# Xharlie/BtcDet

Hardware: AMD Instinct MI355X
Metric: scenes/s fwd+bwd KITTI-Car bs=2/GPU (BtcDet hot path) (higher is better)
Workload: dtype f32

## Files before the change

btcdet_amd/_lib.py:

```python
import ctypes
import os

import numpy as np
import torch

_HERE = os.path.dirname(os.path.abspath(__file__))
LIB_PATH = os.path.join(_HERE, "libbtcdet_hip.so")
_lib = None

c_i32p = ctypes.POINTER(ctypes.c_int32)
c_f32p = ctypes.POINTER(ctypes.c_float)
vp = ctypes.c_void_p
ci = ctypes.c_int
sz = ctypes.c_size_t

MODE_SUBM, MODE_CONV, MODE_TRANSPOSE = 0, 1, 2


class BtcHipError(RuntimeError):
    pass


class BtcOccConfig(ctypes.Structure):
    _fields_ = [("batch", ctypes.c_int32), ("grid", ctypes.c_int32 * 3), ("sphere_grid", ctypes.c_int32 * 3),
# ... 74 lines not shown
    "btc_conv_bf16w_supported": (ci, [ci, ci, ci]),
    "btc_weights_to_bf16": (ci, [vp, ci, ci, ci, vp, vp, vp]),
    "btc_conv_split_supported": (ci, [ci, ci, ci]),
    "btc_set_scratch": (ci, [vp, vp, sz]),
    "btc_conv_split_wanted": (ci, [ci, ci, ci, ci]),
    "btc_weights_split3": (ci, [vp, ci, ci, ci, vp, vp, vp]),
    "btc_weights_split3_multi": (ci, [vp, vp, vp, c_i32p, c_i32p, c_i32p, ci, vp]),
    "btc_weights_to_bf16_multi": (ci, [vp, vp, vp, c_i32p, c_i32p, c_i32p, ci, vp]),
    "btc_conv_fwd_bf16w": (ci, [vp, vp, vp, vp, ci, ci, ci, ci, vp, vp]),
    "btc_conv_dgrad_bf16w": (ci, [vp, vp, vp, ci, ci, ci, ci, vp, vp]),
    "btc_row_orders": (ci, [vp, c_i32p, c_i32p, ci, vp, vp]),
    "btc_row_orders_keyed": (ci, [vp, vp, c_i32p, c_i32p, ci, vp, vp]),
    "btc_conv_apply_ordered": (ci, [ci, ci, vp, vp, vp, vp, vp, ci, ci, ci, ci, vp, vp]),
    "btc_conv_apply_src": (ci, [ci, ci, vp, ctypes.c_longlong, vp, vp, vp, vp, ci, ci, ci, ci, vp, vp]),
    "btc_conv_wgrad_ordered": (ci, [ci, vp, vp, vp, ci, vp, ci, vp, vp, ci, ci, ci, vp, vp, sz, vp]),
    "btc_conv_wgrad_slabs": (ci, [ci, vp, vp, vp, ci, vp, ci, vp, vp, ci, ci, ci, vp, vp, sz, vp, vp]),
    "btc_wgrad_reduce_multi": (ci, [vp, vp, vp, vp, ci, vp]),
    "btc_adam_group_ws_bytes": (sz, [ci]),
    "btc_adam_max_segments": (ci, []),
    "btc_grads_pack": (ci, [vp, ci, vp, vp, vp, vp, c_i32p, vp, vp]),
    "btc_adam_group_step": (ci, [vp, ci, vp, vp, vp, vp, c_i32p, ci, vp, vp, vp, ctypes.c_longlong, ctypes.c_float, ctypes.c_float, ctypes.c_float,
                                 ctypes.c_float, ctypes.c_float, ctypes.c_float, vp, sz, vp]),
    "btc_maxpool_fwd": (ci, [vp, vp, ci, ci, ci, vp, vp]),
    "btc_maxpool_bwd": (ci, [vp, vp, vp, vp, ci, ci, ci, vp, vp]),
    "btc_dense_fwd": (ci, [vp, vp, ci, ci, c_i32p, vp, vp]),
    "btc_dense_bwd": (ci, [vp, vp, ci, ci, c_i32p, vp, vp]),
    "btc_revoxelize_ws_bytes": (sz, [ci, ci, c_i32p]),
    "btc_revoxelize_count": (ci, [vp, ci, ci, c_i32p, vp, vp, vp, sz, vp]),
    "btc_revoxelize_fill": (ci, [vp, vp, ci, ci, ci, c_i32p, ci, ci, vp, vp, vp, vp, sz, vp]),
    "btc_pass_occ_vox_ws_bytes": (sz, [ctypes.POINTER(BtcPovConfig), ci, ci]),
    "btc_pass_occ_vox_count": (ci, [ctypes.POINTER(BtcPovConfig), vp, vp, vp, vp, vp, vp, ci, ci, ci, vp, vp, sz, vp]),
    "btc_pass_occ_vox_fill": (ci, [ctypes.POINTER(BtcPovConfig), vp, ci, ci, ci, ci, ci, ci, vp, vp, vp, vp, vp, vp, sz, vp]),
    "btc_pass_occ_vox_fill_i32": (ci, [ctypes.POINTER(BtcPovConfig), vp, ci, ci, ci, ci, ci, ci, vp, vp, vp, vp, vp, vp, vp, vp, sz, vp]),
    "btc_occ_loss_ws_bytes": (sz, []),
    "btc_occ_loss_fwd": (ci, [vp, vp, vp, vp, vp, vp, vp, vp, ci, ctypes.c_longlong, ctypes.c_float, ctypes.c_float, ctypes.c_float, vp, vp, vp,
                              sz, vp]),
    "btc_occ_loss_bwd": (ci, [vp, vp, vp, vp, vp, vp, vp, vp, ci, ctypes.c_longlong, ctypes.c_float, vp, vp, vp, vp, vp]),
    "btc_occ_loss_fwd_total": (ci, [vp, vp, vp, vp, vp, vp, vp, vp, ci, ctypes.c_longlong, ctypes.c_float, ctypes.c_float, ctypes.c_float, vp, vp,
                                    vp, sz, vp]),
    "btc_occ_loss_bwd_total": (ci, [vp, vp, vp, vp, vp, vp, vp, vp, ci, ctypes.c_longlong, ctypes.c_float, vp, vp, vp, vp, vp]),
    "btc_dense_split_fwd": (ci, [vp, vp, ci, ci, ci, vp, vp, vp, vp]),
    "btc_occ_prob": (ci, [vp, vp, ci, ctypes.c_longlong, vp, vp]),
    "btc_dense_split_bwd": (ci, [vp, vp, vp, ci, ci, ci, vp, vp, vp]),
    "btc_cat_pad_fwd": (ci, [vp, ci, vp, ci, ctypes.c_longlong, ci, ci, vp, vp]),
    "btc_cat_pad_bwd": (ci, [vp, ci, ctypes.c_longlong, ci, vp, ci, vp, ci, vp]),
    "btc_sumsq2_ws_bytes": (sz, []),
    "btc_sumsq2_fwd": (ci, [vp, ctypes.c_longlong, ci, ctypes.c_double, vp, ctypes.c_longlong, ci, ctypes.c_double, vp, vp, sz, vp]),
    "btc_sumsq2_bwd": (ci, [vp, ctypes.c_longlong, ci, ctypes.c_float, vp, vp, ctypes.c_longlong, ci, ctypes.c_float, vp, vp, vp]),
    "btc_bn_ws_bytes": (sz, [ci]),
    "btc_bn_relu_fwd": (ci, [vp, ci, ci, vp, vp, vp, vp, vp, ctypes.c_float, ctypes.c_float, ci, ci, vp, vp, vp, vp, sz, vp]),
    "btc_spin": (ci, [ci, vp]),
    "btc_bn_relu_bwd": (ci, [vp, vp, vp, ci, ci, vp, vp, vp, ci, ci, vp, vp, vp, vp, sz, vp]),
    "btc_bn_relu_fwd_bf16": (ci, [vp, ci, ci, vp, vp, vp, vp, vp, ctypes.c_float, ctypes.c_float, ci, ci, vp, vp, vp, vp, sz, vp]),
    "btc_bn_relu_bwd_bf16": (ci, [vp, vp, vp, ci, ci, vp, vp, vp, ci, ci, vp, vp, vp, vp, sz, vp]),
    "btc_ball_query": (ci, [vp, vp, vp, vp, ci, ci, ctypes.c_float, ctypes.c_float, ci, vp, vp]),
    "btc_group_points": (ci, [vp, vp, vp, vp, ci, ci, ci, ci, vp, vp]),
    "btc_group_points_grad": (ci, [vp, vp, vp, vp, ci, ci, ci, ci, ci, vp, vp]),
    "btc_furthest_point_sampling": (ci, [vp, ci, ci, ci, vp, vp, vp]),
    "btc_three_nn": (ci, [vp, vp, vp, vp, ci, ci, vp, vp, vp]),
    "btc_three_interpolate": (ci, [vp, vp, vp, ci, ci, vp, vp]),
    "btc_three_interpolate_grad": (ci, [vp, vp, vp, ci, ci, ci, vp, vp]),
    "btc_bn_fuse_ws_bytes": (sz, []),
    "btc_conv_bn_relu_fwd": (ci, [ci, vp, vp, vp, vp, vp, ci, ci, ci, ci, vp, vp, vp, vp, vp, vp, ctypes.c_float, ctypes.c_float, ci, vp, vp, vp, vp, sz, vp, vp]),
    "btc_conv_bn_relu_fwd_src": (ci, [ci, vp, ctypes.c_longlong, vp, vp, vp, vp, ci, ci, ci, ci, vp, vp, vp, vp, vp, vp, ctypes.c_float, ctypes.c_float, ci, vp, vp, vp, vp, sz, vp, vp]),
    "btc_col_sum": (ci, [vp, ci, ci, vp, vp, sz, vp]),
    "btc_col_sum_bf16": (ci, [vp, ci, ci, vp, vp, sz, vp]),
    "btc_occ_targets_ws_bytes": (sz, [ctypes.POINTER(BtcOccConfig)]),
    "btc_occ_backproject_lut": (ci, [ctypes.POINTER(BtcOccConfig), vp, vp]),
    "btc_occ_targets": (ci, [ctypes.POINTER(BtcOccConfig), vp, vp, vp, ci, ci, ci, vp, vp, vp, vp, ci, vp, vp,
                             ctypes.POINTER(BtcOccBuffers), vp, sz, vp]),
}

EXPORTED_SYMBOLS = tuple(_SIGS.keys())

_INFER_SIGS = {
    "btc_conv_bn_eval_fwd": (ci, [ci, vp, ctypes.c_longlong, vp, vp, vp, vp, ci, ci, ci, ci, vp, vp, vp, vp, ctypes.c_float, ci, vp, vp]),
    "btc_det_select_nms_ws_bytes": (sz, [ci, ci]),
    "btc_det_select_nms": (ci, [vp, vp, ci, ci, ci, ci, ci, ctypes.c_float, ctypes.c_float, ci, ci, ci, vp, vp, vp, vp, sz, vp]),
    "btc_det_finish": (ci, [vp, vp, ci, ci, ci, ci, ci, ci, vp, vp, vp, vp, ci, vp, ci, ci, vp, ci, ci, c_f32p, ci, vp, vp, vp, vp, vp, vp]),
    "btc_kitti_overlaps": (ci, [vp, vp, vp, vp, vp, c_i32p, ci, vp, vp, vp]),
    "btc_kitti_match_tp": (ci, [vp, vp, vp, vp, vp, vp, vp, c_i32p, ci, ci, ci, ci, ci, ci, vp, vp, vp]),
    "btc_kitti_match_stats_ws_bytes": (sz, [ci, ci, ci, ci, ci]),
    "btc_kitti_match_stats": (ci, [vp, vp, vp, vp, vp, vp, vp, vp, vp, vp, vp, c_i32p, ci, ci, ci, ci, ci, ci, ci, vp, vp, vp, sz, vp]),
}

INFER_EXPORTED_SYMBOLS = tuple(_INFER_SIGS.keys())


def lib():
    global _lib
    if _lib is None:
        if not os.path.exists(LIB_PATH):
            raise BtcHipError(
                f"{LIB_PATH} not found: build it with `python -c 'import __graft_entry__ as g; g.build()'` "
                f"or `make -C btcdet_amd/csrc` (there is no CPU fallback for the hot path)")
        L = ctypes.CDLL(LIB_PATH)
        for name, (res, args) in list(_SIGS.items()) + list(_INFER_SIGS.items()):
            fn = getattr(L, name)
            fn.restype = res
            fn.argtypes = args
        for kv in filter(None, os.environ.get("BTC_TUNE", "").split(",")):
            k, v = kv.split("=")
            if L.btc_tune_set(int(k), int(v)) != 0:
                raise BtcHipError("BTC_TUNE: bad entry %r" % kv)
        _lib = L
    return _lib


_fast = False


def fast():
    global _fast
    if _fast is False:
        _fast = None
        if os.environ.get("BTC_FASTPATH", "1") != "0":
            try:
                lib()
                from . import _btcfast
                if _btcfast.abi_version() == lib().btc_version():
                    _fast = _btcfast
            except ImportError:
                _fast = None
    return _fast


def check(rc, what):
    if rc != 0:
        msg = lib().btc_last_error().decode("utf-8", "replace")
        raise BtcHipError(f"{what} failed (code {rc}): {msg}")


_raw_stream = torch._C._cuda_getCurrentRawStream
_cur_device = torch._C._cuda_getDevice


def stream_ptr():
    return _raw_stream(_cur_device())


def ptr(t):
    if t is None:
        return None
    if not (t.is_cuda and t.is_contiguous()):
        raise BtcHipError("expected a contiguous tensor on the GPU (HIP) device")
    return t.data_ptr()


_I3_CACHE = {}


def i3(v):
    if isinstance(v, (int, np.integer)):
        key = (int(v),) * 3
    else:
        key = tuple(int(x) for x in np.asarray(v).reshape(-1))
        if len(key) != 3:
            raise BtcHipError(f"expected 3 values, got {v!r}")
    a = _I3_CACHE.get(key)
    if a is None:
        a = np.ascontiguousarray(np.array(key, dtype=np.int32))
        a.setflags(write=False)
        a_ptr = a.ctypes.data_as(c_i32p)
        _I3_CACHE[key] = a
        _I3P_CACHE[id(a)] = (a, a_ptr)
    return a
# ... 19 lines not shown
```

btcdet_amd/csrc/btc_common.h:

```cpp
#pragma once
#include <hip/hip_runtime.h>
#include <stdint.h>
#include <stdio.h>

#include "../../include/btcdet_hip.h"

#define BTC_EMPTY_KEY (-1)
#define BTC_EMPTY_IDX 0x7F7F7F7F

void btc_set_error(const char* fmt, ...);

#define BTC_CHECK_ARG(cond, ...)            \
  do {                                      \
    if (!(cond)) {                          \
      btc_set_error(__VA_ARGS__);           \
      return BTC_EINVAL;                    \
    }                                       \
  } while (0)

#define BTC_HIP(call)                                                             \
  do {                                                                            \
    hipError_t e_ = (call);                                                       \
    if (e_ != hipSuccess) {                                                       \
      btc_set_error("%s failed: %s (%s:%d)", #call, hipGetErrorString(e_), __FILE__, __LINE__); \
      return BTC_ELAUNCH;                                                         \
    }                                                                             \
  } while (0)

#define BTC_LAUNCH_CHECK()                                                        \
  do {                                                                            \
    hipError_t e_ = hipGetLastError();                                            \
    if (e_ != hipSuccess) {                                                       \
      btc_set_error("kernel launch failed: %s (%s:%d)", hipGetErrorString(e_), __FILE__, __LINE__); \
      return BTC_ELAUNCH;                                                         \
    }                                                                             \
  } while (0)

#if defined(__HIP_DEVICE_COMPILE__) && !defined(__gfx950__)
#error "the fence-free last-arriver protocol (btc_ticket_take) is derived for gfx950's sc1 write-through stores only"
#endif
#if defined(__HIPCC__)
template <class T>
__device__ __forceinline__ void btc_st_agent(T* p, T v) { __hip_atomic_store(p, v, __ATOMIC_RELAXED, __HIP_MEMORY_SCOPE_AGENT); }
template <class T>
__device__ __forceinline__ T btc_ld_agent(const T* p) { return __hip_atomic_load(p, __ATOMIC_RELAXED, __HIP_MEMORY_SCOPE_AGENT); }
__device__ __forceinline__ int btc_ticket_take(int32_t* counter) {
  asm volatile("s_waitcnt vmcnt(0)" ::: "memory");
  return __hip_atomic_fetch_add(counter, 1, __ATOMIC_RELAXED, __HIP_MEMORY_SCOPE_AGENT);
}
__device__ __forceinline__ void btc_ticket_acquire() { __builtin_amdgcn_fence(__ATOMIC_ACQUIRE, "agent"); }
#endif

#define BTC_TUNE_KEYS 24
int btc_tune_get(int key);

bool btc_apply_glds_supported(int K, int Cred, int Cres);
bool btc_apply_glds_has_shape(int shape, bool bf = false);
size_t btc_apply_glds_lds_bytes(int shape, int kc, int K, bool bf, int stages = 3);
int btc_apply_glds_stages(int shape, int kc, int K, bool bf, int asked);
int btc_launch_apply_glds(bool trans_w, int shape, int kc, int xcd, bool bf, const void* feat, const float* W, const float* bias,
                          const int32_t* nbr, const int32_t* order , int n_rows, int K, int Cred, int Cres, void* out,
                          hipStream_t stream, const struct BnFuse* bn = nullptr );

int btc_apply(const char* who, int pass, int operands, const void* src, long long src_rows, const void* W, const float* bias, const int32_t* nbr,
              const int32_t* order, int n_rows, int K, int Cin, int Cout, void* dst, hipStream_t stream, const struct BnFuse* bn);

int btc_apply_bf16w(const void* src, const void* Wq, const float* bias, const int32_t* nbr, const int32_t* order, int n_rows, int K, int Cred,
                    int Cres, void* dst, hipStream_t stream, int mirror = 0, const struct BnFuse* bn = nullptr);
bool btc_wgrad_x_supported(int mode, int K, int cg, int cc);
int btc_wgrad_x_plan(int mode, int rows, int K, int cg, int cc, int* S, int* ph, int* z = nullptr);
int btc_launch_wgrad_x(int mode, const void* g, const void* c, const int32_t* map, const int32_t* ord, int rows, int K, int cg, int cc, float* part,
                       int swap, hipStream_t stream);
int btc_wgrad_n_kind(int K, int Cin, int Cout);
int btc_wgrad_n_plan(int rows);
int btc_launch_wgrad_n(bool bf, const void* walked, const void* gathered, const int32_t* map, int rows, int K, int Cw, int Cn, float* part,
                       int flags , hipStream_t stream);
constexpr size_t BTC_SCRATCH_HEAD = 64 * 1024;
constexpr long long BTC_SCRATCH_TICKETS = BTC_SCRATCH_HEAD / 4;
void* btc_scratch(hipStream_t stream, size_t* bytes);
struct BnFuse;
int btc_apply_split(const float* src, const void* Ws, const float* bias, const int32_t* nbr, const int32_t* order, int n_rows, int K, int Cred,
                    int Cres, float* dst, hipStream_t stream, int mirror, const BnFuse* bn);

__host__ __device__ __forceinline__ unsigned short btc_f32_to_bf16(float f) {
  union { float f; unsigned u; } c;
  c.f = f;
  unsigned u = c.u;
  if ((u & 0x7fffffffu) > 0x7f800000u) return (unsigned short)((u >> 16) | 0x40);
  u += 0x7fffu + ((u >> 16) & 1u);
  return (unsigned short)(u >> 16);
}
__host__ __device__ __forceinline__ float btc_bf16_to_f32(unsigned short h) {
  union { float f; unsigned u; } c;
  c.u = (unsigned)h << 16;
  return c.f;
}

template <bool BF>
__device__ __forceinline__ float4 btc_ld4(const float* base, size_t i) {
  if (!BF) return *reinterpret_cast<const float4*>(base + i);
  const uint2 v = *reinterpret_cast<const uint2*>(reinterpret_cast<const unsigned short*>(base) + i);
  return make_float4(__uint_as_float(v.x << 16), __uint_as_float(v.x & 0xffff0000u), __uint_as_float(v.y << 16),
                     __uint_as_float(v.y & 0xffff0000u));
}
template <bool BF>
__device__ __forceinline__ float btc_ld1(const float* base, size_t i) {
  if (!BF) return base[i];
  return __uint_as_float((unsigned)reinterpret_cast<const unsigned short*>(base)[i] << 16);
}
template <bool BF>
__device__ __forceinline__ void btc_st4(float* base, size_t i, float a, float b, float c, float d) {
  if (!BF) {
    *reinterpret_cast<float4*>(base + i) = make_float4(a, b, c, d);
  } else {
    uint2 v;
    v.x = (unsigned)btc_f32_to_bf16(a) | ((unsigned)btc_f32_to_bf16(b) << 16);
    v.y = (unsigned)btc_f32_to_bf16(c) | ((unsigned)btc_f32_to_bf16(d) << 16);
    *reinterpret_cast<uint2*>(reinterpret_cast<unsigned short*>(base) + i) = v;
  }
}
template <bool BF>
__device__ __forceinline__ void btc_st1(float* base, size_t i, float a) {
  if (!BF) base[i] = a;
  else reinterpret_cast<unsigned short*>(base)[i] = btc_f32_to_bf16(a);
}

#ifdef __cplusplus
#include <mutex>
constexpr int BTC_MAX_DEVICES = 16;
struct BtcPerDeviceOnce {
  std::once_flag flag[BTC_MAX_DEVICES];
};
template <class F>
static inline void btc_once_per_device(BtcPerDeviceOnce& o, F&& fn) {
  int dev = 0;
  (void)hipGetDevice(&dev);
  std::call_once(o.flag[dev >= 0 && dev < BTC_MAX_DEVICES ? dev : 0], fn);
}
#endif

typedef float f32x4 __attribute__((ext_vector_type(4)));
constexpr int TM = 64;
__host__ __device__ constexpr int ldb_of(int nt) { return nt * 16 + (((nt * 16) % 32 == 0) ? 16 : 0); }

static inline int btc_cdiv(long long a, long long b) { return (int)((a + b - 1) / b); }
static inline size_t btc_align(size_t x, size_t a = 256) { return (x + a - 1) / a * a; }
static inline unsigned btc_pow2_ge(unsigned long long v) {
  unsigned long long p = 1;
// ... 40 lines not shown
```

btcdet_amd/csrc/sparse_conv.hip:

```cpp
#include <mutex>

#include "btc_common.h"
#include "bn_fuse.h"

namespace {

constexpr int KC = 32;
constexpr int LDA = KC + 2;

template <int NT, bool TRANS_W, bool VEC, int KB, int THREADS>
__global__ __launch_bounds__(THREADS) void conv_apply(const float* __restrict__ feat, const float* __restrict__ W,
                                                  const float* __restrict__ bias, const int32_t* __restrict__ nbr,
                                                  int n_rows, int K, int Cred, int Cres, float* __restrict__ out, int mirror, const BnFuse bn) {
  extern __shared__ __attribute__((aligned(16))) char smem[];
  constexpr int TM = THREADS / 4;
  constexpr int LDB = ldb_of(NT);
  constexpr int NB = NT * 512 / THREADS;
  float* As = (float*)smem;
  float* Bs = As + KB * TM * LDA;
  int32_t* s_nbr = (int32_t*)(Bs + KB * KC * LDB);
  int32_t* s_kact = s_nbr + TM * K;
  int32_t* s_nact = s_kact + K;

  const int tid = threadIdx.x, lane = tid & 63, wave = tid >> 6;
  const int row0 = blockIdx.x * TM;
  const int n0 = blockIdx.y * (NT * 16);

  for (int e = tid; e < K; e += THREADS) s_kact[e] = 0;
  __syncthreads();
  {
    const long long gbase = (long long)row0 * K;
    const long long gend = (long long)n_rows * K;
    for (int e = tid; e < TM * K; e += THREADS) {
      const int kk = e % K;
      int v = (gbase + e < gend) ? nbr[mirror ? gbase + e - kk + (K - 1 - kk) : gbase + e] : -1;
      s_nbr[e] = v;
      if (v >= 0) s_kact[kk] = 1;
    }
  }
  __syncthreads();
  if (tid == 0) {
    int n = 0;
    for (int k = 0; k < K; ++k)
      if (s_kact[k]) s_kact[n++] = k;
    *s_nact = n;
  }
  __syncthreads();
  const int n_act = *s_nact;
  const int n_chunks = (KB > 1) ? 1 : (Cred + KC - 1) / KC;
  const int n_items = (KB > 1) ? (n_act + KB - 1) / KB : n_act * n_chunks;

  f32x4 acc[NT];
#pragma unroll
  for (int nt = 0; nt < NT; ++nt) acc[nt] = (f32x4){0.f, 0.f, 0.f, 0.f};
  const int arow = wave * 16 + (lane & 15);
  const int kq = lane >> 4;

  float4 av[KB][2];
  float as_[KB][8];
  float bv[KB][NB];

  int pq = 0, pr = 0, cr = 0;
  auto prefetch = [&](int item) {
    const int pq_now = pq, pr_now = pr;
    if (KB == 1 && ++pr == n_chunks) { pr = 0; ++pq; }
#pragma unroll
    for (int kb = 0; kb < KB; ++kb) {
      const int ai = (KB > 1) ? item * KB + kb : pq_now;
      const bool live = ai < n_act;
      const int k = live ? s_kact[ai] : 0;
      const int cc = (KB > 1) ? 0 : pr_now * KC;
      const int kc = min(KC, Cred - cc);
      const float* Wk = W + (size_t)k * Cred * Cres;
      if (VEC) {
#pragma unroll
        for (int i = 0; i < 2; ++i) {
          int e = i * THREADS + tid, r = e / (KC / 4), c = (e % (KC / 4)) * 4;
          int j = live ? s_nbr[r * K + k] : -1;
          av[kb][i] = (j >= 0 && c < kc) ? *reinterpret_cast<const float4*>(feat + (size_t)j * Cred + cc + c) : make_float4(0.f, 0.f, 0.f, 0.f);
        }
      } else {
#pragma unroll
        for (int i = 0; i < 8; ++i) {
          int e = i * THREADS + tid, r = e / KC, c = e % KC;
          int j = live ? s_nbr[r * K + k] : -1;
// ... 210 lines not shown
      const int col = nt * 16 + lrow;
      const float bv0 = (bias && col < Cres) ? bias[col] : 0.f;
      BnEvalCol ec = {0.f, 0.f, 1.f, 0.f};
      if (ev) ec = bn_eval_col(bn, col);
#pragma unroll
      for (int r = 0; r < 4; ++r) {
        const int row = row0 + kq * 4 + r;
        vals[nt][r] = bias ? (acc[nt][r] + bv0) : acc[nt][r];
        if (ev) vals[nt][r] = bn_affine(vals[nt][r], ec.m, ec.rs, ec.g, ec.b, bn.ev_relu);
        if (col < Cres && row < n_rows) out[(size_t)row * Cres + col] = vals[nt][r];
      }
    }
    if (bn.slots) bn_fuse_wave<NT>(bn, vals, valid, 0, (int)(tile & (bn.nslots - 1)));
    __builtin_amdgcn_wave_barrier();
  }
  if (bn.slots) bn_fuse_finish(bn, (int*)smem, (double*)(smem + 16));
}


__global__ __launch_bounds__(256) void maxpool_fwd_k(const float* __restrict__ feat, const int32_t* __restrict__ nbr,
                                                     int n_out, int K, int C, float* __restrict__ out) {
  long long t = (long long)blockIdx.x * blockDim.x + threadIdx.x;
  if (t >= (long long)n_out * C) return;
  int i = (int)(t / C), c = (int)(t % C);
  float m = 0.f;
  for (int k = 0; k < K; ++k) {
    int j = nbr[(size_t)i * K + k];
    if (j >= 0) m = fmaxf(m, feat[(size_t)j * C + c]);
  }
  out[t] = m;
}

__global__ __launch_bounds__(256) void maxpool_bwd_k(const float* __restrict__ feat, const float* __restrict__ out,
                                                     const float* __restrict__ dout, const int32_t* __restrict__ nbr_in,
                                                     int n_in, int K, int C, float* __restrict__ din) {
  long long t = (long long)blockIdx.x * blockDim.x + threadIdx.x;
  if (t >= (long long)n_in * C) return;
  int j = (int)(t / C), c = (int)(t % C);
  float v = feat[t], g = 0.f;
  for (int k = 0; k < K; ++k) {
    int i = nbr_in[(size_t)j * K + k];
    if (i >= 0 && out[(size_t)i * C + c] == v) g += dout[(size_t)i * C + c];
  }
  din[t] = g;
}

__global__ __launch_bounds__(256) void dense_fwd_k(const float* __restrict__ feat, const int4* __restrict__ idx, int n, int C,
                                                   int D, int H, int Wd, float* __restrict__ dense) {
  long long t = (long long)blockIdx.x * blockDim.x + threadIdx.x;
  if (t >= (long long)n * C) return;
  int c = (int)(t / n), i = (int)(t % n);
  int4 q = idx[i];
  size_t vol = (size_t)D * H * Wd;
  dense[((size_t)q.x * C + c) * vol + ((size_t)q.y * H + q.z) * Wd + q.w] = feat[(size_t)i * C + c];
}

__global__ __launch_bounds__(256) void dense_bwd_k(const float* __restrict__ ddense, const int4* __restrict__ idx, int n, int C,
                                                   int D, int H, int Wd, float* __restrict__ dfeat) {
  long long t = (long long)blockIdx.x * blockDim.x + threadIdx.x;
  if (t >= (long long)n * C) return;
  int c = (int)(t / n), i = (int)(t % n);
  int4 q = idx[i];
  size_t vol = (size_t)D * H * Wd;
  dfeat[(size_t)i * C + c] = ddense[((size_t)q.x * C + c) * vol + ((size_t)q.y * H + q.z) * Wd + q.w];
}

template <int NT, bool TRANS_W, int THREADS>
void launch_apply_t(dim3 grid, size_t lds, hipStream_t stream, bool vec, const float* feat, const float* W, const float* bias,
                    const int32_t* nbr, int n_rows, int K, int Cred, int Cres, float* out, int mirror, const BnFuse& bn) {
  if (lds > 64 * 1024) {
    static BtcPerDeviceOnce once;
    btc_once_per_device(once, [] {
      (void)hipFuncSetAttribute((const void*)conv_apply<NT, TRANS_W, true, 1, THREADS>, hipFuncAttributeMaxDynamicSharedMemorySize, 160 * 1024);
      (void)hipFuncSetAttribute((const void*)conv_apply<NT, TRANS_W, false, 1, THREADS>, hipFuncAttributeMaxDynamicSharedMemorySize, 160 * 1024);
    });
  }
  if (vec) conv_apply<NT, TRANS_W, true, 1, THREADS><<<grid, THREADS, lds, stream>>>(feat, W, bias, nbr, n_rows, K, Cred, Cres, out, mirror, bn);
  else conv_apply<NT, TRANS_W, false, 1, THREADS><<<grid, THREADS, lds, stream>>>(feat, W, bias, nbr, n_rows, K, Cred, Cres, out, mirror, bn);
}

template <bool TRANS_W>
int launch_apply(const float* feat, const float* W, const float* bias, const int32_t* nbr, int n_rows, int K, int Cred,
                 int Cres, float* out, hipStream_t stream, bool bf = false, const int32_t* order = nullptr, int mirror = 0,
                 const BnFuse* bn_ = nullptr) {
  const BnFuse bn = bn_ ? *bn_ : btc_bn_fuse_none();
  if (n_rows <= 0) return BTC_OK;
  BTC_CHECK_ARG(!bf || btc_apply_glds_supported(K, Cred, Cres),
                "bf16 activations need channel counts that are multiples of 16 (K=%d, %d -> %d): convert to fp32", K, Cred, Cres);
  int nt = Cres <= 16 ? 1 : (Cres <= 32 ? 2 : (Cres <= 64 ? 4 : 8));
  const int t_kernel = btc_tune_get(BTC_TUNE_APPLY_KERNEL), t_nt = btc_tune_get(BTC_TUNE_APPLY_NT),
            t_xcd = btc_tune_get(BTC_TUNE_APPLY_XCD);
  if (bf || (t_kernel != 1 && btc_apply_glds_supported(K, Cred, Cres) && (t_kernel == 2 || n_rows < 100000 || (Cred >= 64 && Cres >= 64)))) {
    int shape, kc = (Cred % 64 == 0) ? 64 : ((Cred % 32 == 0) ? 32 : 16);
    if (bf) {
      if (Cres % 128 == 0) shape = 424;
      else if (Cres % 64 == 0) shape = n_rows < 8192 ? 141 : 422;
      else if (Cres % 32 == 0) shape = 221;
      else shape = 411;
    } else if (Cres % 128 == 0) {
      shape = n_rows < 7000 ? 222 : (n_rows < 13000 ? 242 : (n_rows <= 16384 ? 424 : (n_rows < 19500 ? 242 : 424)));
    } else if (Cres % 64 == 0) {
      if (kc == 64) shape = n_rows < 11000 ? 141 : 241;
      else shape = n_rows < 13000 ? 141 : 222;
    } else if (Cres % 32 == 0) {
      shape = 221;
    } else {
      shape = 411;
    }
    if (t_nt > 8 && !bf) {
      int wc = (t_nt / 10) % 10, ntw = t_nt % 10;
      while (ntw > 1 && Cres % (16 * wc * ntw)) ntw >>= 1;
      while (wc > 1 && Cres % (16 * wc * ntw)) wc >>= 1;
      const int cand = (t_nt / 100) * 100 + wc * 10 + ntw;
      if (btc_apply_glds_has_shape(cand)) shape = cand;
    }
    const int t_kc = btc_tune_get(BTC_TUNE_APPLY_KC);
    if (t_kc && Cred % t_kc == 0) kc = t_kc;
    while (kc > 16 && btc_apply_glds_lds_bytes(shape, kc, K, bf) > 160 * 1024) kc >>= 1;
    return btc_launch_apply_glds(TRANS_W, shape, kc, (t_xcd == 2 ? 1 : 0) | (mirror ? 2 : 0), bf, feat, W, bias, nbr, order, n_rows, K, Cred, Cres, out, stream, &bn);
  }
  if (t_kernel != 1 && Cred <= 4 * WS_Q && Cres <= 32 && K <= 64 && n_rows >= 2048 && ws_lds_bytes(K, Cred, nt) <= 160 * 1024) {
    const int n_tiles16 = btc_cdiv(n_rows, 16);
    int wgs = btc_cdiv(n_tiles16, WS_WAVES);
    if (wgs > 256) wgs = 256;
    size_t lds = ws_lds_bytes(K, Cred, nt);
    if (bn.slots && lds < 16 + (size_t)16 * WS_WAVES * 64) lds = 16 + (size_t)16 * WS_WAVES * 64;
    static BtcPerDeviceOnce once;
    btc_once_per_device(once, [] {
      (void)hipFuncSetAttribute((const void*)conv_apply_ws<1, TRANS_W>, hipFuncAttributeMaxDynamicSharedMemorySize, 160 * 1024);
      (void)hipFuncSetAttribute((const void*)conv_apply_ws<2, TRANS_W>, hipFuncAttributeMaxDynamicSharedMemorySize, 160 * 1024);
    });
    if constexpr (!TRANS_W) {
      if (bn.ev_mean) {
        static BtcPerDeviceOnce once_ev;
        btc_once_per_device(once_ev, [] {
          (void)hipFuncSetAttribute((const void*)conv_apply_ws<1, false, true>, hipFuncAttributeMaxDynamicSharedMemorySize, 160 * 1024);
          (void)hipFuncSetAttribute((const void*)conv_apply_ws<2, false, true>, hipFuncAttributeMaxDynamicSharedMemorySize, 160 * 1024);
        });
        if (nt == 1) conv_apply_ws<1, false, true><<<wgs, WS_WAVES * 64, lds, stream>>>(feat, W, bias, nbr, n_rows, K, Cred, Cres, out, mirror, bn);
        else conv_apply_ws<2, false, true><<<wgs, WS_WAVES * 64, lds, stream>>>(feat, W, bias, nbr, n_rows, K, Cred, Cres, out, mirror, bn);
        BTC_LAUNCH_CHECK();
        return BTC_OK;
      }
    }
    if (nt == 1) conv_apply_ws<1, TRANS_W><<<wgs, WS_WAVES * 64, lds, stream>>>(feat, W, bias, nbr, n_rows, K, Cred, Cres, out, mirror, bn);
    else conv_apply_ws<2, TRANS_W><<<wgs, WS_WAVES * 64, lds, stream>>>(feat, W, bias, nbr, n_rows, K, Cred, Cres, out, mirror, bn);
    BTC_LAUNCH_CHECK();
    return BTC_OK;
  }
  const int tm = 64;
  const int n_tiles = btc_cdiv(n_rows, tm);
  while (nt > 2 && (long long)n_tiles * btc_cdiv(Cres, nt * 16) < 512) nt >>= 1;
  if (t_nt && t_nt <= 8) nt = t_nt;
  dim3 grid(n_tiles, btc_cdiv(Cres, nt * 16));
  size_t lds = (size_t)(tm * LDA + KC * ldb_of(nt)) * sizeof(float) + (size_t)(tm * K + K + 1) * sizeof(int32_t);
  const bool vec = (Cred & 3) == 0;
#define BTC_APPLY(NT_) launch_apply_t<NT_, TRANS_W, 256>(grid, lds, stream, vec, feat, W, bias, nbr, n_rows, K, Cred, Cres, out, mirror, bn)
  switch (nt) {
    case 1: BTC_APPLY(1); break;
    case 2: BTC_APPLY(2); break;
    case 4: BTC_APPLY(4); break;
    default: BTC_APPLY(8); break;
  }
#undef BTC_APPLY
  BTC_LAUNCH_CHECK();
  return BTC_OK;
}

int split_source_ok(const char* who, long long src_rows, int Cred) {
  BTC_CHECK_ARG(src_rows >= 0, "%s: BTC_OPERANDS_F32_SPLIT needs the row count of src (btc_conv_apply_src / btc_conv_bn_relu_fwd_src)", who);
  BTC_CHECK_ARG(src_rows * Cred * 4 < 0xFFFFFF00LL, "%s: a source of %lld rows x %d channels is past the 32-bit gather offsets of the split-operand "
                "kernel (4 GB): use BTC_OPERANDS_F32", who, src_rows, Cred);
  return BTC_OK;
}

}

int btc_apply(const char* who, int pass, int operands, const void* src, long long src_rows, const void* W, const float* bias, const int32_t* nbr,
              const int32_t* order, int n_rows, int K, int Cin, int Cout, void* dst, hipStream_t stream, const BnFuse* bn) {
  BTC_CHECK_ARG((pass == BTC_PASS_FWD || pass == BTC_PASS_DGRAD || pass == BTC_PASS_DGRAD_MIRROR) && operands >= BTC_OPERANDS_F32 &&
                    operands <= BTC_OPERANDS_F32_SPLIT, "%s: pass=%d operands=%d", who, pass, operands);
  const int mirror = pass == BTC_PASS_DGRAD_MIRROR;
  const bool fwd = pass == BTC_PASS_FWD;
  BTC_CHECK_ARG(K <= BTC_CONV_K_MAX, "%s: K=%d offsets, more than BTC_CONV_K_MAX = %d", who, K, BTC_CONV_K_MAX);
  BTC_CHECK_ARG(K >= 1 && Cin >= 1 && Cout >= 1 && n_rows >= 0, "%s: bad sizes", who);
  BTC_CHECK_ARG(fwd || bias == nullptr, "%s: dgrad takes no bias", who);
  BTC_CHECK_ARG(!bn || Cout <= BN_FUSE_CMAX, "%s: more than %d channels", who, BN_FUSE_CMAX);
  const int Cred = fwd ? Cin : Cout, Cres = fwd ? Cout : Cin;
  if (operands == BTC_OPERANDS_BF16) {
    const bool ok = btc_conv_bf16w_supported(K, Cred, Cres);
    if (bn) BTC_CHECK_ARG(ok, "%s: bf16 operands need K <= 64, Cin %% 32 == 0, Cout %% 16 == 0", who);
    else BTC_CHECK_ARG(ok, "%s: bf16 operands need K <= 64, Cred %% 32 == 0, Cres %% 16 == 0 (K=%d, %d -> %d)", who, K, Cin, Cout);
    return btc_apply_bf16w(src, W, bias, nbr, order, n_rows, K, Cred, Cres, dst, stream, mirror, bn);
  }
  if (operands == BTC_OPERANDS_F32_SPLIT) {
    if (n_rows > 0) {
      const int rc = split_source_ok(who, src_rows, Cred);
      if (rc) return rc;
    }
    return btc_apply_split((const float*)src, W, bias, nbr, order, n_rows, K, Cred, Cres, (float*)dst, stream, mirror, bn);
  }
  const bool bf = operands == BTC_OPERANDS_BF16_ACT;
  if (fwd) return launch_apply<false>((const float*)src, (const float*)W, bias, nbr, n_rows, K, Cred, Cres, (float*)dst, stream, bf, order, 0, bn);
  return launch_apply<true>((const float*)src, (const float*)W, nullptr, nbr, n_rows, K, Cred, Cres, (float*)dst, stream, bf, order, mirror, bn);
}

#define BTC_SIZES_OK(who, n) BTC_CHECK_ARG(K >= 1 && Cin >= 1 && Cout >= 1 && (n) >= 0, who ": bad sizes")

extern "C" int btc_conv_fwd(const float* feat, const float* W, const float* bias, const int32_t* nbr_out, int n_out, int K,
                            int Cin, int Cout, float* out, void* stream) {
  BTC_SIZES_OK("btc_conv_fwd", n_out);
  return btc_apply("btc_conv_fwd", BTC_PASS_FWD, BTC_OPERANDS_F32, feat, -1LL, W, bias, nbr_out, nullptr, n_out, K, Cin, Cout, out, (hipStream_t)stream, nullptr);
}

extern "C" int btc_conv_dgrad(const float* dout, const float* W, const int32_t* nbr_in, int n_in, int K, int Cin, int Cout,
                              float* din, void* stream) {
  BTC_SIZES_OK("btc_conv_dgrad", n_in);
  return btc_apply("btc_conv_dgrad", BTC_PASS_DGRAD, BTC_OPERANDS_F32, dout, -1LL, W, nullptr, nbr_in, nullptr, n_in, K, Cin, Cout, din, (hipStream_t)stream, nullptr);
}

extern "C" int btc_conv_fwd_bf16(const void* feat, const float* W, const float* bias, const int32_t* nbr_out, int n_out, int K,
                                 int Cin, int Cout, void* out, void* stream) {
  BTC_SIZES_OK("btc_conv_fwd_bf16", n_out);
  if (n_out == 0) return BTC_OK;
  return btc_apply("btc_conv_fwd_bf16", BTC_PASS_FWD, BTC_OPERANDS_BF16_ACT, feat, -1LL, W, bias, nbr_out, nullptr, n_out, K, Cin, Cout, out, (hipStream_t)stream, nullptr);
}

extern "C" int btc_conv_dgrad_bf16(const void* dout, const float* W, const int32_t* nbr_in, int n_in, int K, int Cin, int Cout,
                                   void* din, void* stream) {
  BTC_SIZES_OK("btc_conv_dgrad_bf16", n_in);
  if (n_in == 0) return BTC_OK;
  return btc_apply("btc_conv_dgrad_bf16", BTC_PASS_DGRAD, BTC_OPERANDS_BF16_ACT, dout, -1LL, W, nullptr, nbr_in, nullptr, n_in, K, Cin, Cout, din, (hipStream_t)stream, nullptr);
}
#undef BTC_SIZES_OK

extern "C" int btc_conv_fwd_bf16w(const void* feat, const void* wt_bf16, const float* bias, const int32_t* nbr_out, int n_out, int K, int Cin,
                                  int Cout, void* out, void* stream) {
  BTC_CHECK_ARG(n_out >= 0 && btc_conv_bf16w_supported(K, Cin, Cout), "btc_conv_fwd_bf16w: needs K <= 64, Cin %% 32 == 0, Cout %% 16 == 0 (K=%d, %d -> %d)",
                K, Cin, Cout);
  if (n_out == 0) return BTC_OK;
  return btc_apply("btc_conv_fwd_bf16w", BTC_PASS_FWD, BTC_OPERANDS_BF16, feat, -1LL, wt_bf16, bias, nbr_out, nullptr, n_out, K, Cin, Cout, out, (hipStream_t)stream, nullptr);
}

extern "C" int btc_conv_dgrad_bf16w(const void* dout, const void* w_bf16, const int32_t* nbr_in, int n_in, int K, int Cin, int Cout, void* din,
                                    void* stream) {
  BTC_CHECK_ARG(n_in >= 0 && btc_conv_bf16w_supported(K, Cout, Cin), "btc_conv_dgrad_bf16w: needs K <= 64, Cout %% 32 == 0, Cin %% 16 == 0 (K=%d, %d -> %d)",
                K, Cin, Cout);
  if (n_in == 0) return BTC_OK;
  return btc_apply("btc_conv_dgrad_bf16w", BTC_PASS_DGRAD, BTC_OPERANDS_BF16, dout, -1LL, w_bf16, nullptr, nbr_in, nullptr, n_in, K, Cin, Cout, din, (hipStream_t)stream, nullptr);
}

extern "C" int btc_conv_apply_ordered(int pass, int operands, const void* src, const void* W, const float* bias, const int32_t* nbr,
                                      const int32_t* order, int n_rows, int K, int Cin, int Cout, void* dst, void* stream) {
  return btc_apply("btc_conv_apply_ordered", pass, operands, src, pass == BTC_PASS_DGRAD_MIRROR ? (long long)n_rows : -1LL, W, bias, nbr, order, n_rows,
                   K, Cin, Cout, dst, (hipStream_t)stream, nullptr);
}

extern "C" int btc_conv_apply_src(int pass, int operands, const void* src, long long src_rows, const void* W, const float* bias, const int32_t* nbr,
                                  const int32_t* order, int n_rows, int K, int Cin, int Cout, void* dst, void* stream) {
  return btc_apply("btc_conv_apply_src", pass, operands, src, src_rows, W, bias, nbr, order, n_rows, K, Cin, Cout, dst, (hipStream_t)stream, nullptr);
}

extern "C" int btc_maxpool_fwd(const float* feat, const int32_t* nbr_out, int n_out, int K, int C, float* out, void* stream) {
  if (n_out <= 0) return BTC_OK;
  maxpool_fwd_k<<<btc_cdiv((long long)n_out * C, 256), 256, 0, (hipStream_t)stream>>>(feat, nbr_out, n_out, K, C, out);
  BTC_LAUNCH_CHECK();
  return BTC_OK;
}

extern "C" int btc_maxpool_bwd(const float* feat, const float* out, const float* dout, const int32_t* nbr_in, int n_in, int K,
                               int C, float* din, void* stream) {
  if (n_in <= 0) return BTC_OK;
  maxpool_bwd_k<<<btc_cdiv((long long)n_in * C, 256), 256, 0, (hipStream_t)stream>>>(feat, out, dout, nbr_in, n_in, K, C, din);
  BTC_LAUNCH_CHECK();
  return BTC_OK;
}

extern "C" int btc_dense_fwd(const float* feat, const int32_t* indices, int n, int C, const int32_t* h_shape, float* dense,
                             void* stream) {
  if (n <= 0) return BTC_OK;
  dense_fwd_k<<<btc_cdiv((long long)n * C, 256), 256, 0, (hipStream_t)stream>>>(feat, (const int4*)indices, n, C, h_shape[0],
                                                                               h_shape[1], h_shape[2], dense);
  BTC_LAUNCH_CHECK();
  return BTC_OK;
}

extern "C" int btc_dense_bwd(const float* ddense, const int32_t* indices, int n, int C, const int32_t* h_shape, float* dfeat,
// ... 8 lines not shown
```

include/btcdet_hip_infer.h:

```cpp
#ifndef BTCDET_HIP_INFER_H
#define BTCDET_HIP_INFER_H

#include <stddef.h>
#include <stdint.h>

#include "btcdet_hip.h"

#ifdef __cplusplus
extern "C" {
#endif

int btc_conv_bn_eval_fwd(int operands, const void* src, long long src_rows, const void* W, const float* bias, const int32_t* nbr,
                         const int32_t* order, int n_rows, int K, int Cin, int Cout, const float* gamma, const float* beta,
                         const float* running_mean, const float* running_var, float eps, int relu, void* y, void* stream);

size_t btc_det_select_nms_ws_bytes(int batch, int n);
int btc_det_select_nms(const float* cls_preds, const float* box_preds, int batch, int n, int num_class, int box_stride, int normalized,
                       float score_thresh, float nms_thresh, int rotated, int pre_max, int post_max, long long* keep, int32_t* num_keep,
                       int32_t* best_class, void* ws, size_t ws_bytes, void* stream);

int btc_det_finish(const float* cls_preds, const float* box_preds, int batch, int n, int num_class, int box_stride, int normalized,
                   int raw_score, const long long* keep, const int32_t* num_keep, const int32_t* best_class, const long long* labels,
                   int post_max, const float* gt_boxes, int n_gt, int gt_stride, const float* rois, int n_rois, int roi_stride,
                   const float* h_thresh, int n_thresh, float* pred_boxes, float* pred_scores, long long* pred_labels, float* pred_iou,
                   long long* counters, void* stream);

int btc_kitti_overlaps(const double* gt_rows, const double* dt_rows, const double* dc_boxes, const int32_t* frames, const long long* pairs,
                       const int32_t* h_frames, int n_frames, double* ov, double* ov_dc, void* stream);

int btc_kitti_match_tp(const double* ov, const double* dt_rows, const int8_t* ign_gt, const int8_t* ign_dt, const double* min_overlaps,
                       const int32_t* frames, const long long* pairs, const int32_t* h_frames, int n_frames, int metric_first, int n_metric,
                       int n_class, int n_diff, int n_level, int32_t* tp_det, int32_t* tp_count, void* stream);
size_t btc_kitti_match_stats_ws_bytes(int n_frames, int n_class, int n_diff, int n_level, int compute_aos);
int btc_kitti_match_stats(const double* ov, const double* ov_dc, const double* gt_rows, const double* dt_rows, const int8_t* ign_gt,
                          const int8_t* ign_dt, const double* min_overlaps, const double* thresholds, const int32_t* n_thresholds,
                          const int32_t* frames, const long long* pairs, const int32_t* h_frames, int n_frames, int metric_first, int n_metric,
                          int n_class, int n_diff, int n_level, int compute_aos, int32_t* counts, double* similarity, void* ws,
                          size_t ws_bytes, void* stream);

#ifdef __cplusplus
}
#endif
#endif
```

Measured before the change: 581.8.

## Add narrow-output sparse conv apply kernels for fwd and dgrad with family dispatch

Adds dedicated MFMA kernels for sparse conv shapes with at most 8 output channels (forward) or narrow dgrad. The forward kernel keeps W in LDS, double-buffers neighbour-map loads and the buffer-load gathers, and transposes the gathered data with permlane swaps. The dgrad kernel keeps the weights in registers. Kernel selection moves into a shared btc_apply_family function, which is also exported for querying. This targets the poor utilisation of the wide WS/staged paths on narrow layers such as the heads. It relies on 32-bit buffer offsets, gated by the source row count.

Measured after the change: 583.7, median of 4. About the same (+0.3%).

```diff
diff --git a/btcdet_amd/_lib.py b/btcdet_amd/_lib.py
--- a/btcdet_amd/_lib.py
+++ b/btcdet_amd/_lib.py
@@ -180,6 +180,7 @@
     "btc_kitti_match_tp": (ci, [vp, vp, vp, vp, vp, vp, vp, c_i32p, ci, ci, ci, ci, ci, ci, vp, vp, vp]),
     "btc_kitti_match_stats_ws_bytes": (sz, [ci, ci, ci, ci, ci]),
     "btc_kitti_match_stats": (ci, [vp, vp, vp, vp, vp, vp, vp, vp, vp, vp, vp, c_i32p, ci, ci, ci, ci, ci, ci, ci, vp, vp, vp, sz, vp]),
+    "btc_conv_apply_family": (ci, [ci, ci, ci, ci, ci, ci, ci]),
 }
 
 INFER_EXPORTED_SYMBOLS = tuple(_INFER_SIGS.keys())
diff --git a/btcdet_amd/csrc/btc_common.h b/btcdet_amd/csrc/btc_common.h
--- a/btcdet_amd/csrc/btc_common.h
+++ b/btcdet_amd/csrc/btc_common.h
@@ -64,6 +64,11 @@
 
 int btc_apply(const char* who, int pass, int operands, const void* src, long long src_rows, const void* W, const float* bias, const int32_t* nbr,
               const int32_t* order, int n_rows, int K, int Cin, int Cout, void* dst, hipStream_t stream, const struct BnFuse* bn);
+
+int btc_apply_family(int pass, int operands, long long src_rows, int n_rows, int K, int Cin, int Cout, bool with_bn);
+int btc_launch_apply_n(bool fwd, const float* src, const float* W, const float* bias, const int32_t* nbr, int n_rows, int K, int Cin, int Cout,
+                       float* dst, int mirror, hipStream_t stream);
+bool btc_apply_ws_ok(int K, int Cred, int Cres);
 
 int btc_apply_bf16w(const void* src, const void* Wq, const float* bias, const int32_t* nbr, const int32_t* order, int n_rows, int K, int Cred,
                     int Cres, void* dst, hipStream_t stream, int mirror = 0, const struct BnFuse* bn = nullptr);
diff --git a/btcdet_amd/csrc/conv_apply_n.hip b/btcdet_amd/csrc/conv_apply_n.hip
--- /dev/null
+++ b/btcdet_amd/csrc/conv_apply_n.hip
@@ -0,0 +1,279 @@
+#include "btc_common.h"
+#include "../../include/btcdet_hip_infer.h"
+
+typedef unsigned nu32x4 __attribute__((ext_vector_type(4)));
+
+namespace {
+
+#define N_RECORDS 0xFFFFFF00u
+constexpr int NF_WAVES = 16;
+constexpr int ND_WAVES = 4;
+constexpr int N_MR = 16;
+constexpr int N_CUS = 256;
+constexpr int ROW_GATE = 2048;
+
+__host__ __device__ inline size_t nf_lds_bytes(int K, int Cred) {
+  return (size_t)K * Cred * 8 * sizeof(float) + (size_t)NF_WAVES * 16 * K * sizeof(int32_t);
+}
+
+__device__ __forceinline__ void load_map(const int32_t* __restrict__ nbr, int tile, int n_tiles, int n_rows, int K, int lane, int (&mr)[N_MR]) {
+  const long long gbase = (long long)tile * 16 * K, gend = (long long)n_rows * K;
+#pragma unroll
+  for (int u = 0; u < N_MR; ++u) {
+    const int e = u * 64 + lane;
+    mr[u] = (tile < n_tiles && e < 16 * K && gbase + e < gend) ? nbr[gbase + e] : -1;
+  }
+}
+__device__ __forceinline__ void store_map(int32_t* nb, int K, int lane, const int (&mr)[N_MR]) {
+#pragma unroll
+  for (int u = 0; u < N_MR; ++u) {
+    const int e = u * 64 + lane;
+    if (e < 16 * K) nb[e] = mr[u];
+  }
+}
+
+__device__ __forceinline__ void transpose4(const nu32x4 v, float (&t)[4]) {
+  const auto a = __builtin_amdgcn_permlane32_swap(v.x, v.z, false, false);
+  const auto b = __builtin_amdgcn_permlane32_swap(v.y, v.w, false, false);
+  const auto c = __builtin_amdgcn_permlane16_swap(a[0], b[0], false, false);
+  const auto d = __builtin_amdgcn_permlane16_swap(a[1], b[1], false, false);
+  t[0] = __uint_as_float(c[0]);
+  t[1] = __uint_as_float(c[1]);
+  t[2] = __uint_as_float(d[0]);
+  t[3] = __uint_as_float(d[1]);
+}
+
+template <int NL>
+__global__ __launch_bounds__(NF_WAVES * 64) void conv_apply_nf(const float* __restrict__ feat, const float* __restrict__ W, const float* __restrict__ bias,
+                                                              const int32_t* __restrict__ nbr, int n_rows, int K, int Cres, float* __restrict__ out) {
+  extern __shared__ __attribute__((aligned(16))) char smem[];
+  constexpr int Cred = NL * 16;
+  constexpr int KB = NL == 1 ? 4 : (NL == 2 ? 3 : (NL == 3 ? 2 : 1));
+  float* Ws = (float*)smem;
+  int32_t* nb_all = (int32_t*)(Ws + (size_t)K * Cred * 8);
+  const int tid = threadIdx.x, lane = tid & 63, kq = lane >> 4, lrow = lane & 15;
+  const int wave = __builtin_amdgcn_readfirstlane(tid >> 6);
+  int32_t* nb = nb_all + wave * 16 * K;
+
+  for (int e = tid; e < K * Cred * 8; e += NF_WAVES * 64) {
+    const int c = e & 7;
+    Ws[e] = c < Cres ? W[(size_t)(e >> 3) * Cres + c] : 0.f;
+  }
+  __syncthreads();
+
+  const __amdgpu_buffer_rsrc_t rf = __builtin_amdgcn_make_buffer_rsrc((void*)feat, 0, N_RECORDS, 0x00020000);
+  const int n_tiles = (n_rows + 15) >> 4;
+  const int stride = gridDim.x * NF_WAVES;
+  const float bv0 = (bias && lrow < Cres) ? bias[lrow] : 0.f;
+  const float* Wl = Ws + (lrow & 7);
+
+  int mr[N_MR];
+  int tile = blockIdx.x * NF_WAVES + wave;
+  load_map(nbr, tile, n_tiles, n_rows, K, lane, mr);
+  while (tile < n_tiles) {
+    store_map(nb, K, lane, mr);
+    __builtin_amdgcn_wave_barrier();
+    load_map(nbr, tile + stride, n_tiles, n_rows, K, lane, mr);
+
+    f32x4 acc = (f32x4){0.f, 0.f, 0.f, 0.f};
+    nu32x4 v[2][KB][NL];
+    auto fetch = [&](int set, int k0) {
+#pragma unroll
+      for (int g = 0; g < KB; ++g) {
+        const int k = k0 + g;
+        const int j = k < K ? nb[lrow * K + k] : -1;
+        const unsigned base = (unsigned)j * (unsigned)(Cred * 4) + (unsigned)kq * 16u, dead = (unsigned)(j >> 31);
+#pragma unroll
+        for (int l = 0; l < NL; ++l) v[set][g][l] = __builtin_amdgcn_raw_buffer_load_b128(rf, (base + 64u * l) | dead, 0, 0);
+      }
+    };
+    auto math = [&](int set, int k0) {
+#pragma unroll
+      for (int g = 0; g < KB; ++g) {
+        const int k = k0 + g;
+        if (k >= K) break;
+        const float* Wk = Wl + (size_t)k * Cred * 8;
+#pragma unroll
+        for (int l = 0; l < NL; ++l) {
+          float t[4];
+          transpose4(v[set][g][l], t);
+#pragma unroll
+          for (int c = 0; c < 4; ++c) {
+            const float w = Wk[(16 * l + 4 * c + kq) * 8];
+            acc = __builtin_amdgcn_mfma_f32_16x16x4f32(t[c], lrow < 8 ? w : 0.f, acc, 0, 0, 0);
+          }
+        }
+      }
+    };
+    fetch(0, 0);
+    for (int k0 = 0; k0 < K; k0 += 2 * KB) {
+      fetch(1, k0 + KB);
+      math(0, k0);
+      if (k0 + KB >= K) break;
+      fetch(0, k0 + 2 * KB);
+      math(1, k0 + KB);
+    }
+
+    if (lrow < Cres) {
+#pragma unroll
+      for (int r = 0; r < 4; ++r) {
+        const int row = (tile << 4) + kq * 4 + r;
+        if (row < n_rows) out[(size_t)row * Cres + lrow] = bias ? (acc[r] + bv0) : acc[r];
+      }
+    }
+    __builtin_amdgcn_wave_barrier();
+    tile += stride;
+  }
+}
+
+template <int NT, int NS>
+__global__ __launch_bounds__(ND_WAVES * 64, 2) void conv_apply_nd(const float* __restrict__ dy, const float* __restrict__ W, const int32_t* __restrict__ nbr,
+                                                                 int n_rows, int K, int Cy, int Cres, float* __restrict__ out, int mirror) {
+  __shared__ int32_t nb_all[ND_WAVES][16 * 64 + 1];
+  const int tid = threadIdx.x, lane = tid & 63, kq = lane >> 4, lrow = lane & 15;
+  const int wave = __builtin_amdgcn_readfirstlane(tid >> 6);
+  int32_t* nb = nb_all[wave];
+  const int n0 = blockIdx.y * (NT * 16);
+  const int n_cols = K * Cy;
+  const __amdgpu_buffer_rsrc_t ry = __builtin_amdgcn_make_buffer_rsrc((void*)dy, 0, N_RECORDS, 0x00020000);
+
+  unsigned pk[NS];
+  float wreg[NS][NT];
+#pragma unroll
+  for (int s = 0; s < NS; ++s) {
+    const int c = 4 * s + kq;
+    const bool live = c < n_cols;
+    const int kk = live ? c / Cy : 0, co = c - kk * Cy;
+    pk[s] = (unsigned)(live ? lrow * K + (mirror ? K - 1 - kk : kk) : 16 * K) | ((unsigned)co << 16);
+#pragma unroll
+    for (int nt = 0; nt < NT; ++nt) wreg[s][nt] = live ? W[((size_t)kk * Cres + n0 + nt * 16 + lrow) * Cy + co] : 0.f;
+  }
+  if (lane == 0) nb[16 * K] = -1;
+
+  const int n_tiles = (n_rows + 15) >> 4;
+  const int stride = gridDim.x * ND_WAVES;
+  int tile = blockIdx.x * ND_WAVES + wave;
+  int mr[N_MR];
+  float a[2][NS];
+  auto gather = [&](int set) {
+#pragma unroll
+    for (int s = 0; s < NS; ++s) {
+      if (4 * s >= n_cols) break;
+      unsigned p = pk[s];
+      asm volatile("" : "+v"(p));
+      const int j = nb[p & 0xFFFFu];
+      a[set][s] = __uint_as_float(__builtin_amdgcn_raw_buffer_load_b32(ry, (((unsigned)j * (unsigned)Cy + (p >> 16)) << 2) | (unsigned)(j >> 31), 0, 0));
+    }
+  };
+  auto stage = [&](int set, int t) {
+    store_map(nb, K, lane, mr);
+    __builtin_amdgcn_wave_barrier();
+    load_map(nbr, t + stride, n_tiles, n_rows, K, lane, mr);
+    gather(set);
+    __builtin_amdgcn_wave_barrier();
+  };
+  auto finish = [&](int set, int t) {
+    f32x4 acc[NT];
+#pragma unroll
+    for (int nt = 0; nt < NT; ++nt) acc[nt] = (f32x4){0.f, 0.f, 0.f, 0.f};
+#pragma unroll
+    for (int s = 0; s < NS; ++s) {
+      if (4 * s >= n_cols) break;
+#pragma unroll
+      for (int nt = 0; nt < NT; ++nt) acc[nt] = __builtin_amdgcn_mfma_f32_16x16x4f32(a[set][s], wreg[s][nt], acc[nt], 0, 0, 0);
+    }
+#pragma unroll
+    for (int nt = 0; nt < NT; ++nt)
+#pragma unroll
+      for (int r = 0; r < 4; ++r) {
+        const int row = (t << 4) + kq * 4 + r;
+        if (row < n_rows) out[(size_t)row * Cres + n0 + nt * 16 + lrow] = acc[nt][r];
+      }
+  };
+
+  load_map(nbr, tile, n_tiles, n_rows, K, lane, mr);
+  if (tile < n_tiles) {
+    stage(0, tile);
+    for (;;) {
+      stage(1, tile + stride);
+      finish(0, tile);
+      tile += stride;
+      if (tile >= n_tiles) break;
+      stage(0, tile + stride);
+      finish(1, tile);
+      tile += stride;
+      if (tile >= n_tiles) break;
+    }
+  }
+}
+
+bool narrow_fwd_ok(int K, int Cin, int Cout) {
+  return Cout <= 8 && Cin >= 16 && Cin <= 64 && (Cin & 15) == 0 && K <= 64 && nf_lds_bytes(K, Cin) <= 160 * 1024;
+}
+bool narrow_dgrad_ok(int K, int Cin, int Cout) { return Cout <= 8 && K * Cout <= 176 && Cin >= 16 && Cin <= 64 && (Cin & 15) == 0 && K <= 64; }
+
+}
+
+int btc_apply_family(int pass, int operands, long long src_rows, int n_rows, int K, int Cin, int Cout, bool with_bn) {
+  if (operands == BTC_OPERANDS_BF16) return BTC_APPLY_FAMILY_BF16;
+  if (operands == BTC_OPERANDS_F32_SPLIT) return BTC_APPLY_FAMILY_SPLIT;
+  const bool bf = operands == BTC_OPERANDS_BF16_ACT, fwd = pass == BTC_PASS_FWD;
+  const int Cred = fwd ? Cin : Cout, Cres = fwd ? Cout : Cin;
+  const int t_kernel = btc_tune_get(BTC_TUNE_APPLY_KERNEL);
+  if (bf || (t_kernel != 1 && btc_apply_glds_supported(K, Cred, Cres) && (t_kernel == 2 || n_rows < 100000 || (Cred >= 64 && Cres >= 64))))
+    return BTC_APPLY_FAMILY_GLDS;
+  if (t_kernel == 1) return BTC_APPLY_FAMILY_STAGED;
+  const long long reach = src_rows > n_rows ? src_rows : n_rows;
+  if (!with_bn && n_rows >= ROW_GATE && reach * Cred * 4 < (long long)N_RECORDS) {
+    if (fwd && narrow_fwd_ok(K, Cin, Cout)) return BTC_APPLY_FAMILY_NARROW_FWD;
+    if (!fwd && narrow_dgrad_ok(K, Cin, Cout)) return BTC_APPLY_FAMILY_NARROW_DGRAD;
+  }
+  if (btc_apply_ws_ok(K, Cred, Cres) && n_rows >= ROW_GATE) return BTC_APPLY_FAMILY_WS;
+  return BTC_APPLY_FAMILY_STAGED;
+}
+
+extern "C" int btc_conv_apply_family(int pass, int operands, int n_rows, int K, int Cin, int Cout, int with_bn) {
+  BTC_CHECK_ARG((pass == BTC_PASS_FWD || pass == BTC_PASS_DGRAD || pass == BTC_PASS_DGRAD_MIRROR) && operands >= BTC_OPERANDS_F32 &&
+                    operands <= BTC_OPERANDS_F32_SPLIT && K >= 1 && Cin >= 1 && Cout >= 1 && n_rows >= 0,
+                "btc_conv_apply_family: pass=%d operands=%d, K=%d, %d -> %d, %d rows", pass, operands, K, Cin, Cout, n_rows);
+  return btc_apply_family(pass, operands, -1LL, n_rows, K, Cin, Cout, with_bn != 0);
+}
+
+int btc_launch_apply_n(bool fwd, const float* src, const float* W, const float* bias, const int32_t* nbr, int n_rows, int K, int Cin, int Cout,
+                       float* dst, int mirror, hipStream_t stream) {
+  BTC_CHECK_ARG(fwd ? narrow_fwd_ok(K, Cin, Cout) : narrow_dgrad_ok(K, Cin, Cout), "btc_launch_apply_n: unsupported shape K=%d, %d -> %d", K, Cin, Cout);
+  if (n_rows <= 0) return BTC_OK;
+  const int n_tiles = btc_cdiv(n_rows, 16);
+  if (fwd) {
+    int wgs = btc_cdiv(n_tiles, NF_WAVES);
+    if (wgs > N_CUS) wgs = N_CUS;
+    const size_t lds = nf_lds_bytes(K, Cin);
+    static BtcPerDeviceOnce once;
+    btc_once_per_device(once, [] {
+      (void)hipFuncSetAttribute((const void*)conv_apply_nf<1>, hipFuncAttributeMaxDynamicSharedMemorySize, 160 * 1024);
+      (void)hipFuncSetAttribute((const void*)conv_apply_nf<2>, hipFuncAttributeMaxDynamicSharedMemorySize, 160 * 1024);
+      (void)hipFuncSetAttribute((const void*)conv_apply_nf<3>, hipFuncAttributeMaxDynamicSharedMemorySize, 160 * 1024);
+      (void)hipFuncSetAttribute((const void*)conv_apply_nf<4>, hipFuncAttributeMaxDynamicSharedMemorySize, 160 * 1024);
+    });
+#define NF_LAUNCH(NL_) conv_apply_nf<NL_><<<wgs, NF_WAVES * 64, lds, stream>>>(src, W, bias, nbr, n_rows, K, Cout, dst)
+    switch (Cin >> 4) {
+      case 1: NF_LAUNCH(1); break;
+      case 2: NF_LAUNCH(2); break;
+      case 3: NF_LAUNCH(3); break;
+      default: NF_LAUNCH(4); break;
+    }
+#undef NF_LAUNCH
+  } else {
+    const bool wide = K * Cout > 136, two = (Cin & 31) == 0 && !wide;
+    int wgs = btc_cdiv(n_tiles, ND_WAVES);
+    if (wgs > 2 * N_CUS) wgs = 2 * N_CUS;
+    dim3 grid(wgs, Cin / (two ? 32 : 16));
+#define ND_LAUNCH(NT_, NS_) conv_apply_nd<NT_, NS_><<<grid, ND_WAVES * 64, 0, stream>>>(src, W, nbr, n_rows, K, Cout, Cin, dst, mirror)
+    if (two) ND_LAUNCH(2, 34);
+    else if (!wide) ND_LAUNCH(1, 34);
+    else ND_LAUNCH(1, 44);
+#undef ND_LAUNCH
+  }
+  BTC_LAUNCH_CHECK();
+  return BTC_OK;
+}
diff --git a/btcdet_amd/csrc/sparse_conv.hip b/btcdet_amd/csrc/sparse_conv.hip
--- a/btcdet_amd/csrc/sparse_conv.hip
+++ b/btcdet_amd/csrc/sparse_conv.hip
@@ -1,6 +1,7 @@
 #include <mutex>
 
 #include "btc_common.h"
+#include "../../include/btcdet_hip_infer.h"
 #include "bn_fuse.h"
 
 namespace {
@@ -377,15 +378,16 @@
 template <bool TRANS_W>
 int launch_apply(const float* feat, const float* W, const float* bias, const int32_t* nbr, int n_rows, int K, int Cred,
                  int Cres, float* out, hipStream_t stream, bool bf = false, const int32_t* order = nullptr, int mirror = 0,
-                 const BnFuse* bn_ = nullptr) {
+                 const BnFuse* bn_ = nullptr, long long src_rows = -1) {
   const BnFuse bn = bn_ ? *bn_ : btc_bn_fuse_none();
   if (n_rows <= 0) return BTC_OK;
   BTC_CHECK_ARG(!bf || btc_apply_glds_supported(K, Cred, Cres),
                 "bf16 activations need channel counts that are multiples of 16 (K=%d, %d -> %d): convert to fp32", K, Cred, Cres);
   int nt = Cres <= 16 ? 1 : (Cres <= 32 ? 2 : (Cres <= 64 ? 4 : 8));
-  const int t_kernel = btc_tune_get(BTC_TUNE_APPLY_KERNEL), t_nt = btc_tune_get(BTC_TUNE_APPLY_NT),
-            t_xcd = btc_tune_get(BTC_TUNE_APPLY_XCD);
-  if (bf || (t_kernel != 1 && btc_apply_glds_supported(K, Cred, Cres) && (t_kernel == 2 || n_rows < 100000 || (Cred >= 64 && Cres >= 64)))) {
+  const int t_nt = btc_tune_get(BTC_TUNE_APPLY_NT), t_xcd = btc_tune_get(BTC_TUNE_APPLY_XCD);
+  const int family = btc_apply_family(TRANS_W ? (mirror ? BTC_PASS_DGRAD_MIRROR : BTC_PASS_DGRAD) : BTC_PASS_FWD, bf ? BTC_OPERANDS_BF16_ACT : BTC_OPERANDS_F32,
+                                      src_rows, n_rows, K, TRANS_W ? Cres : Cred, TRANS_W ? Cred : Cres, bn_ != nullptr);
+  if (family == BTC_APPLY_FAMILY_GLDS) {
     int shape, kc = (Cred % 64 == 0) ? 64 : ((Cred % 32 == 0) ? 32 : 16);
     if (bf) {
       if (Cres % 128 == 0) shape = 424;
@@ -414,7 +416,9 @@
     while (kc > 16 && btc_apply_glds_lds_bytes(shape, kc, K, bf) > 160 * 1024) kc >>= 1;
     return btc_launch_apply_glds(TRANS_W, shape, kc, (t_xcd == 2 ? 1 : 0) | (mirror ? 2 : 0), bf, feat, W, bias, nbr, order, n_rows, K, Cred, Cres, out, stream, &bn);
   }
-  if (t_kernel != 1 && Cred <= 4 * WS_Q && Cres <= 32 && K <= 64 && n_rows >= 2048 && ws_lds_bytes(K, Cred, nt) <= 160 * 1024) {
+  if (family == BTC_APPLY_FAMILY_NARROW_FWD || family == BTC_APPLY_FAMILY_NARROW_DGRAD)
+    return btc_launch_apply_n(!TRANS_W, feat, W, bias, nbr, n_rows, K, TRANS_W ? Cres : Cred, TRANS_W ? Cred : Cres, out, mirror, stream);
+  if (family == BTC_APPLY_FAMILY_WS) {
     const int n_tiles16 = btc_cdiv(n_rows, 16);
     int wgs = btc_cdiv(n_tiles16, WS_WAVES);
     if (wgs > 256) wgs = 256;
@@ -462,6 +466,14 @@
   return BTC_OK;
 }
 
+}
+
+bool btc_apply_ws_ok(int K, int Cred, int Cres) {
+  return Cred <= 4 * WS_Q && Cres <= 32 && K <= 64 && ws_lds_bytes(K, Cred, Cres <= 16 ? 1 : 2) <= 160 * 1024;
+}
+
+namespace {
+
 int split_source_ok(const char* who, long long src_rows, int Cred) {
   BTC_CHECK_ARG(src_rows >= 0, "%s: BTC_OPERANDS_F32_SPLIT needs the row count of src (btc_conv_apply_src / btc_conv_bn_relu_fwd_src)", who);
   BTC_CHECK_ARG(src_rows * Cred * 4 < 0xFFFFFF00LL, "%s: a source of %lld rows x %d channels is past the 32-bit gather offsets of the split-operand "
@@ -496,8 +508,8 @@
     return btc_apply_split((const float*)src, W, bias, nbr, order, n_rows, K, Cred, Cres, (float*)dst, stream, mirror, bn);
   }
   const bool bf = operands == BTC_OPERANDS_BF16_ACT;
-  if (fwd) return launch_apply<false>((const float*)src, (const float*)W, bias, nbr, n_rows, K, Cred, Cres, (float*)dst, stream, bf, order, 0, bn);
-  return launch_apply<true>((const float*)src, (const float*)W, nullptr, nbr, n_rows, K, Cred, Cres, (float*)dst, stream, bf, order, mirror, bn);
+  if (fwd) return launch_apply<false>((const float*)src, (const float*)W, bias, nbr, n_rows, K, Cred, Cres, (float*)dst, stream, bf, order, 0, bn, src_rows);
+  return launch_apply<true>((const float*)src, (const float*)W, nullptr, nbr, n_rows, K, Cred, Cres, (float*)dst, stream, bf, order, mirror, bn, src_rows);
 }
 
 #define BTC_SIZES_OK(who, n) BTC_CHECK_ARG(K >= 1 && Cin >= 1 && Cout >= 1 && (n) >= 0, who ": bad sizes")
diff --git a/include/btcdet_hip_infer.h b/include/btcdet_hip_infer.h
--- a/include/btcdet_hip_infer.h
+++ b/include/btcdet_hip_infer.h
@@ -38,6 +38,15 @@
                           int n_class, int n_diff, int n_level, int compute_aos, int32_t* counts, double* similarity, void* ws,
                           size_t ws_bytes, void* stream);
 
+#define BTC_APPLY_FAMILY_STAGED 0
+#define BTC_APPLY_FAMILY_GLDS 1
+#define BTC_APPLY_FAMILY_WS 2
+#define BTC_APPLY_FAMILY_NARROW_FWD 3
+#define BTC_APPLY_FAMILY_NARROW_DGRAD 4
+#define BTC_APPLY_FAMILY_BF16 5
+#define BTC_APPLY_FAMILY_SPLIT 6
+int btc_conv_apply_family(int pass, int operands, int n_rows, int K, int Cin, int Cout, int with_bn);
+
 #ifdef __cplusplus
 }
 #endif
```
